# placrosse/Zaru

Measured on AMD Instinct MI355X. Metric: end-to-end faces/sec (detect+468-pt mesh), 1080p synthetic, 1/2/4/8 GPU, higher is better.
Workload: dtype f32

## Files before the change

zaru_amd/csrc/kernels/fused.hip:

```cpp
#include <algorithm>
#include <cstdio>
#include <cstdlib>

#include "../runtime/zr_kernels.h"
#include "act.h"
#include "epilogue.h"
#include "lds_dma.h"
#include "sample.h"

namespace zr {


typedef float f32x2 __attribute__((ext_vector_type(2)));
typedef float f32x4 __attribute__((ext_vector_type(4)));

constexpr int STH = 8, STW = 32;

template <int K, int S, int CO, bool PRE>
__global__ __launch_bounds__(256) void stem_kernel(const StemParams P) {
    constexpr int RIN = (STH - 1) * S + K, WIN = (STW - 1) * S + K;
    __shared__ float patch[3][RIN][WIN];
    const int tiles_x = (P.OW + STW - 1) / STW;
    const int ty0 = (blockIdx.x / tiles_x) * STH, tx0 = (blockIdx.x % tiles_x) * STW;
    const int n = blockIdx.y;
// ... 476 lines not shown
    static const bool v16 = [] {
        const char *e = std::getenv("ZARU_HIP_VALU16_VF8");
        return !e || std::strtol(e, nullptr, 10) != 0;
    }();
    const bool small = db && !((CO == 32 || (CO == 16 && v16 && p.in.W >= 96 && p.g.K >= 32)) && fit8);
    const int vf = small ? 4 : VFKC;
    const int bufsz = buf_of(vf);
    dim3 grid((ntiles + 7) / 8 * 8);
    if (db && vres) return dwpw_vres_go<K, S, CO>(p, s);
    if (db) {
        const size_t lds = 2 * sizeof(float) * (size_t)bufsz;
        if (small)
            hipLaunchKernelGGL((dwpw_valu_kernel<K, S, CO, true, 4>), grid, dim3(256), lds, s, p, tpi, ntiles, bufsz, lw);
        else
            hipLaunchKernelGGL((dwpw_valu_kernel<K, S, CO, true, VFKC>), grid, dim3(256), lds, s, p, tpi, ntiles, bufsz, lw);
    } else {
        const size_t lds = sizeof(float) * (size_t)VFKC * rmax * lw;
        hipLaunchKernelGGL((dwpw_valu_kernel<K, S, CO, false, VFKC>), grid, dim3(256), lds, s, p, tpi, ntiles, bufsz, lw);
    }
    const int vfe = db ? vf : VFKC;
    return kernel_name("dwpw_valu_kernel<%d,%d,%d,%s,%d>", K, S, CO, db ? "true" : "false", vfe);
}

template <int K, int S>
const char *dwpw_valu_co(const DwPwParams &p, hipStream_t s) {
    if (p.g.M <= 16) return dwpw_valu_go<K, S, 16>(p, s);
    if (p.g.M <= 32) return dwpw_valu_go<K, S, 32>(p, s);
    if (p.g.M <= 48) return dwpw_valu_go<K, S, 48>(p, s);
    return dwpw_valu_go<K, S, 64>(p, s);
}

}

static bool valu_form(const DwPwParams &p) {
    if (!form_on(FORM_VALU) || p.g.P < VTQ || p.in.W % 4 != 0 || p.in.W > 248 || p.g.M > 48 || p.g.K * p.g.M > 2048)
        return false;
    if (p.g.ncols % p.g.P != 0) return false;
    const int rows = (VTQ / p.OW + 2) * p.stride + p.k;
    return sizeof(float) * (size_t)VFKC * rows * (p.in.W + 8) <= 64 * 1024;
}

bool dwpw_is_vres1(const DwPwParams &p) {
    if (!valu_form(p) || p.stride != 1 || p.g.M > 32 || !form_on(FORM_VALU_DB)) return false;
    const int P = p.g.P, tpi = (P + VTQ - 1) / VTQ;
    int rmax = 0;
    for (int t = 0; t < tpi; t++) {
        const int q0 = t * VTQ, a = q0 / p.OW, b = std::min(q0 + VTQ - 1, P - 1) / p.OW;
        rmax = std::max(rmax, b - a + p.k);
    }
    const size_t buf4 = (size_t)(4 * rmax * (p.in.W + 8) + 255) / 256 * 256;
    return 2 * sizeof(float) * buf4 <= 64 * 1024 && vres_mode(p, 1, p.g.M <= 16 ? 16 : 32) == 1;
}

const char *launch_dwpw(const DwPwParams &p, hipStream_t s) {
    if (valu_form(p)) {
        if (p.k == 3) return p.stride == 1 ? dwpw_valu_co<3, 1>(p, s) : dwpw_valu_co<3, 2>(p, s);
        return p.stride == 1 ? dwpw_valu_co<5, 1>(p, s) : dwpw_valu_co<5, 2>(p, s);
    }
    return launch_dwpw_mfma(p, s);
}

const char *launch_dwpw_group(const DwPwParams *p, int n, hipStream_t s) {
    for (int i = 0; i < n; ++i)
        if (valu_form(p[i])) return nullptr;
    return launch_dwpw_mfma_group(p, n, s);
}

}
```

zaru_amd/csrc/kernels/misc.hip:

```cpp
#include <algorithm>
#include <cstdarg>
#include <cstdio>
#include <cstdlib>
#include <mutex>
#include <set>
#include <string>
#include "../runtime/zr_kernels.h"
#include "act.h"

namespace zr {

const char *kernel_name(const char *fmt, ...) {
    char buf[128];
    va_list ap;
    va_start(ap, fmt);
    vsnprintf(buf, sizeof buf, fmt, ap);
    va_end(ap);
    static std::mutex mu;
    static std::set<std::string> names;
    std::lock_guard<std::mutex> g(mu);
    return names.insert(buf).first->c_str();
}

bool form_on(Form f) {
    static const unsigned mask = [] {
        static const char *const names[FORM_COUNT] = {"dma", "v4", "valu", "valu_db", "rows", "vres", "vstore", "ws", "groups", "dwgap", "rt", "ir", "irl", "irl2", "bneck", "pin", "stemblock"};
        unsigned m = (1u << FORM_COUNT) - 1;
        const char *e = std::getenv("ZARU_HIP_FORMS");
        for (std::string s = e ? e : ""; !s.empty();) {
            const size_t comma = s.find(',');
            const std::string tok = s.substr(0, comma);
            s = comma == std::string::npos ? "" : s.substr(comma + 1);
            if (tok.size() < 2 || (tok[0] != '+' && tok[0] != '-')) continue;
            for (int i = 0; i < FORM_COUNT; i++)
                if (tok.compare(1, std::string::npos, names[i]) == 0)
                    m = tok[0] == '+' ? m | (1u << i) : m & ~(1u << i);
        }
        return m;
    }();
    return (mask >> f) & 1u;
}

__device__ __forceinline__ const float *plane_ptr(const Plane &p, int n, int c) {
    return p.p + (int64_t)n * p.sN + (int64_t)c * p.sC;
}

__global__ __launch_bounds__(256) void elt_kernel(const EltParams P) {
    const int plane = blockIdx.x;
    const int c = plane / P.N, n = plane - c * P.N;
    const int HW = P.H * P.W;
    float *dst = P.out + (int64_t)n * P.o_sN + (int64_t)c * P.o_sC;
    for (int q = blockIdx.y * blockDim.x + threadIdx.x; q < HW; q += gridDim.y * blockDim.x) {
        float v;
        if (P.op == 0) {
            v = plane_ptr(P.a, n, c)[q];
        } else if (P.op == 1) {
            v = plane_ptr(P.a, n, c)[q] + plane_ptr(P.b, n, c)[q];
        } else if (P.op == 2) {
            const int y = q / P.W, x = q - y * P.W;
            const float *s = plane_ptr(P.a, n, c) + (int64_t)(2 * y) * P.a.W + 2 * x;
            v = fmaxf(fmaxf(s[0], s[1]), fmaxf(s[P.a.W], s[P.a.W + 1]));
        } else {
            v = c < P.a.C ? plane_ptr(P.a, n, c)[q] : 0.f;
        }
        dst[q] = apply_act(P.act, v, c);
    }
}

const char *launch_elt(const EltParams &p, hipStream_t s) {
    const int HW = p.H * p.W;
    dim3 grid(p.C * p.N, std::min((HW + 255) / 256, 64));
    hipLaunchKernelGGL(elt_kernel, grid, dim3(256), 0, s, p);
    return "elt_kernel";
}

__global__ __launch_bounds__(256) void resize_kernel(const ResizeParams P) {
    const int plane = blockIdx.x;
    const int c = plane / P.N, n = plane - c * P.N;
    if (P.nact && n >= *P.nact) return;
// ... 208 lines not shown
```

zaru_amd/csrc/runtime/plan.cpp:

```cpp
#include "plan.h"

#include <algorithm>
#include <cmath>
#include <cstdlib>
#include <cstring>
#include <map>
#include <set>

namespace zr {
namespace {

struct Val {
    std::vector<int64_t> shape;
    int tensor = -1;
    int lazy = 0;
    std::string lazy_src;
    int step = -1;
    int consumers = 0;
    bool is_input = false;
    int out_idx = -1;
    int64_t out_off = 0;
    bool nhwc = false;
};

// ... 6 lines not shown
int64_t round_up(int64_t v, int64_t m) { return (v + m - 1) / m * m; }

class Compiler {
  public:
    Compiler(const OnnxModel &m, Plan &p, std::string &e) : M(m), P(p), err(e) {}

    bool run(const std::vector<uint32_t> &sel);

  private:
    const OnnxModel &M;
    Plan &P;
    std::string &err;
    std::map<std::string, Val> vals;
    std::map<std::string, int> producer;
    std::set<int> layout_nodes;
    std::vector<bool> needed;

    bool fail(const std::string &s) {
        err = s;
        return false;
    }
    const OnnxTensor *init(const std::string &n) const {
        auto it = M.inits.find(n);
        return it == M.inits.end() ? nullptr : &it->second;
    }
    Val &val(const std::string &n) { return vals[n]; }

    bool infer_shapes();
    bool trace_output(const std::string &name, int oi, int64_t off, bool nhwc);
    bool lower();
    bool lower_conv(const OnnxNode &nd);
    bool lower_gemm_node(const OnnxNode &nd);
    bool lower_act(const OnnxNode &nd);
    bool lower_add(const OnnxNode &nd);
    bool ensure_tensor(const std::string &name);
    TRef ref_of(const std::string &name);
    TRef out_ref(const std::string &name, int C, int H, int W);
    int new_storage(int64_t per_img) {
        P.storage_size.push_back(per_img);
        return (int)P.storage_size.size() - 1;
    }
    int64_t push_weights(const std::vector<float> &w) {
        int64_t off = (int64_t)P.weights.size();
        P.weights.insert(P.weights.end(), w.begin(), w.end());
        while (P.weights.size() % 4) P.weights.push_back(0.f);
        return off;
    }
    bool act_from_node(const OnnxNode &nd, int C, int Cpad, ActDesc &a);
    void finalize_outputs();
    void fuse_dw_gap();
    void group_siblings();
    void mark_inverted_residuals();
    void mark_stem_blocks();
    void allocate();
};

bool Compiler::infer_shapes() {
    for (auto &vi : M.inputs) {
        Val &v = val(vi.name);
        v.shape = vi.dims;
        if (!v.shape.empty() && v.shape[0] <= 0) v.shape[0] = 1;
        v.is_input = true;
    }
    for (auto &kv : M.inits) {
        const OnnxTensor &t = kv.second;
        if (t.dtype == 1 && (int64_t)t.f.size() != t.numel()) return fail("initializer " + kv.first + ": no f32 data");
        val(kv.first).shape = t.dims;
    }
    for (auto &vi : M.inputs)
        for (size_t i = 1; i < vi.dims.size(); i++)
            if (vi.dims[i] <= 0 || vi.dims[i] > (1 << 16)) return fail("graph input " + vi.name + ": bad dims");
    auto weight = [&](const std::string &n, size_t rank) -> const OnnxTensor * {
        const OnnxTensor *t = init(n);
        if (!t || t->dtype != 1 || t->dims.size() != rank) return nullptr;
        for (auto d : t->dims)
            if (d <= 0) return nullptr;
        return t;
    };
    for (size_t ni = 0; ni < M.nodes.size(); ni++) {
        const OnnxNode &nd = M.nodes[ni];
        const std::string &op = nd.op;
        const size_t arity = (op == "Conv" || op == "Add" || op == "PRelu" || op == "Gemm" ||
                              op == "Reshape") ? 2 : 1;
        if (nd.in.size() < arity || nd.out.empty() || nd.in[0].empty())
            return fail(op + " " + nd.name + ": missing operands");
        for (auto &i : nd.in)
            if (!i.empty() && !init(i) && (!vals.count(i) || vals[i].shape.empty()))
                return fail(op + " " + nd.name + ": operand " + i + " is not defined before use");
        for (auto &o : nd.out) producer[o] = (int)ni;
        for (auto &i : nd.in)
            if (!i.empty()) vals[i].consumers++;
        auto in = [&](int k) -> std::vector<int64_t> & { return val(nd.in[k]).shape; };
        std::vector<int64_t> s;
        if (op == "Conv") {
            auto &x = in(0);
            const OnnxTensor *w = weight(nd.in[1], 4);
            if (!w || x.size() != 4) return fail("Conv " + nd.name + ": unsupported operands");
            auto st = nd.getints("strides", {1, 1});
            auto pads = nd.getints("pads", {0, 0, 0, 0});
            const int64_t g = nd.geti("group", 1);
            if (st.size() != 2 || st[0] <= 0 || st[1] <= 0 || pads.size() != 4 ||
                *std::min_element(pads.begin(), pads.end()) < 0 || g <= 0 || x[1] != w->dims[1] * g ||
                w->dims[0] % g)
                return fail("Conv " + nd.name + ": bad strides/pads/group");
            if (nd.in.size() > 2 && !nd.in[2].empty()) {
                const OnnxTensor *b = weight(nd.in[2], 1);
// ... 707 lines not shown
    for (size_t gi = 0; gi < P.steps.size(); ++gi) {
        Step &g = P.steps[gi];
        if (g.kind != S_GAP || g.in.kind != 0 || g.in.c_off != 0) continue;
        int prod = -1, readers = 0;
        for (size_t i = 0; i < P.steps.size(); ++i) {
            const Step &s = P.steps[i];
            if (s.out.kind == 0 && s.out.id == g.in.id) prod = prod < 0 ? (int)i : -2;
            for (const TRef *r : {&s.in, &s.in2})
                if (r->kind == 0 && r->id == g.in.id) ++readers;
        }
        if (prod < 0 || readers != 1) continue;
        Step &d = P.steps[prod];
        if (d.kind != S_DW || (d.kh != 3 && d.kh != 5) || d.kh != d.kw || (int64_t)d.in.H * d.in.W > 512) continue;
        d.kind = S_DWGAP;
        d.dw_oh = d.out.H;
        d.dw_ow = d.out.W;
        d.name += "+" + g.name;
        d.out = g.out;
        d.bytes = 4.0 * ((double)d.in.C * d.in.H * d.in.W + d.in.C);
        P.steps.erase(P.steps.begin() + gi);
        --gi;
    }
}

void Compiler::mark_inverted_residuals() {
    std::vector<int> reads(P.storage_size.size(), 0);
    for (const Step &s : P.steps)
        for (const TRef *r : {&s.in, &s.in2})
            if (r->kind == 0 && r->id >= 0) reads[r->id]++;
    for (size_t i = 0; i + 1 < P.steps.size(); i++) {
        Step &e = P.steps[i];
        const Step &d = P.steps[i + 1];
        e.ir = e.kind == S_GEMM && e.group == 1 && d.group == 1 && e.KK == 1 && e.res_mode == 0 && e.out.kind == 0 &&
               e.out.c_off == 0 && e.in.kind == 0 && e.in.c_off == 0 && d.kind == S_DWPW && d.in.kind == 0 &&
               d.in.id == e.out.id && d.in.c_off == 0 && reads[e.out.id] == 1 && e.M == d.K;
    }
}

void Compiler::mark_stem_blocks() {
    std::vector<int> reads(P.storage_size.size(), 0);
    for (const Step &s : P.steps)
        for (const TRef *r : {&s.in, &s.in2})
            if (r->kind == 0 && r->id >= 0) reads[r->id]++;
    for (size_t i = 0; i + 1 < P.steps.size(); i++) {
        Step &e = P.steps[i];
        const Step &d = P.steps[i + 1];
        e.sb = e.kind == S_DIRECT && e.stem && e.M <= 32 && e.group == 1 && d.group == 1 && e.out.kind == 0 &&
               e.out.c_off == 0 && d.kind == S_DWPW && d.in.kind == 0 && d.in.id == e.out.id && d.in.c_off == 0 &&
               d.res_mode != 0 && d.in2.kind == 0 && d.in2.id == e.out.id && d.in2.c_off == 0 &&
               reads[e.out.id] == 2;
    }
}

void Compiler::group_siblings() {
    const int n = (int)P.steps.size();
    if (n < 2) return;
    auto touches = [](const TRef &r, const TRef &w) {
        return r.kind == w.kind && r.kind != 1 && r.id >= 0 && r.id == w.id;
    };
    std::vector<std::vector<char>> dep(n, std::vector<char>(n, 0));
    for (int j = 0; j < n; ++j)
        for (int i = 0; i < j; ++i) {
            const Step &a = P.steps[i], &b = P.steps[j];
            bool d = touches(b.in, a.out) || touches(b.out, a.out) || touches(b.out, a.in);
            if (b.res_mode || b.kind == S_ELT) d = d || touches(b.in2, a.out);
            if (a.res_mode || a.kind == S_ELT) d = d || touches(b.out, a.in2);
            dep[j][i] = d;
        }
    std::vector<std::vector<char>> anc = dep;
    for (int j = 0; j < n; ++j)
        for (int i = 0; i < j; ++i)
            if (anc[j][i])
                for (int k = 0; k < i; ++k) anc[j][k] |= anc[i][k];
    auto related = [&](int a, int b) { return a < b ? anc[b][a] : anc[a][b]; };
    std::vector<char> done(n, 0);
    auto ready = [&](int j) {
        if (done[j]) return false;
        for (int i = 0; i < j; ++i)
            if (dep[j][i] && !done[i]) return false;
        return true;
    };
    auto future_partner = [&](int s) {
        for (int t = 0; t < n; ++t)
            if (t != s && !done[t] && !ready(t) && !related(s, t) && groupable(P.steps[s], P.steps[t])) return true;
        return false;
    };
    std::vector<Step> out;
    out.reserve(n);
    for (int left = n; left > 0;) {
        std::vector<int> rd;
        for (int j = 0; j < n; ++j)
            if (ready(j)) rd.push_back(j);
        auto partners_of = [&](int s) {
            std::vector<int> g{s};
            for (int t : rd)
                if (t != s && (int)g.size() < ZR_GROUP_MAX && groupable(P.steps[s], P.steps[t])) g.push_back(t);
            return g;
        };
        std::vector<int> g = partners_of(rd[0]);
        if (g.size() == 1 && future_partner(rd[0]))
            for (int r : rd)
                if (r != rd[0] && !future_partner(r)) {
                    g = partners_of(r);
                    break;
                }
        for (size_t k = 0; k < g.size(); ++k) {
            Step st = P.steps[g[k]];
            st.group = k == 0 ? (int)g.size() : 0;
            out.push_back(std::move(st));
            done[g[k]] = 1;
        }
        left -= (int)g.size();
    }
    P.steps = std::move(out);
}

void Compiler::allocate() {
    const size_t ns = P.storage_size.size();
    std::vector<int> first(ns, 1 << 30), last(ns, -1);
    int time = -1;
    std::vector<int> tof(P.steps.size());
    for (size_t i = 0; i < P.steps.size(); i++) {
        const Step &s = P.steps[i];
        if (s.group != 0) ++time;
        tof[i] = time;
        for (const TRef *r : {&s.in, &s.in2, &s.out})
            if (r->kind == 0 && r->id >= 0) {
                first[r->id] = std::min(first[r->id], time);
                last[r->id] = std::max(last[r->id], time);
            }
    }
    for (size_t i = 0; i + 1 < P.steps.size(); i++) {
        if (!P.steps[i].ir && !P.steps[i].sb) continue;
        const TRef &x = P.steps[i].in, &o = P.steps[i + 1].out;
        if (x.kind == 0 && x.id >= 0) last[x.id] = std::max(last[x.id], tof[i + 1]);
        if (o.kind == 0 && o.id >= 0) first[o.id] = std::min(first[o.id], tof[i]);
    }
    std::vector<int> order(ns);
    for (size_t i = 0; i < ns; i++) order[i] = (int)i;
    std::sort(order.begin(), order.end(),
              [&](int a, int b) { return P.storage_size[a] > P.storage_size[b]; });
    P.storage_off.assign(ns, 0);
    std::vector<int> placed;
    int64_t arena = 0;
    for (int id : order) {
        if (last[id] < 0) continue;
        std::vector<std::pair<int64_t, int64_t>> busy;
        for (int o : placed)
            if (!(last[o] < first[id] || last[id] < first[o]))
                busy.push_back({P.storage_off[o], P.storage_off[o] + P.storage_size[o]});
        std::sort(busy.begin(), busy.end());
        int64_t off = 0;
        for (auto &b : busy) {
            if (off + P.storage_size[id] <= b.first) break;
            off = std::max(off, round_up(b.second, 64));
        }
        P.storage_off[id] = off;
        arena = std::max(arena, off + P.storage_size[id]);
        placed.push_back(id);
    }
    P.arena_per_image = round_up(arena, 64);
}

bool Compiler::run(const std::vector<uint32_t> &sel) {
    if (M.inputs.size() != 1) return fail("CNN plans take exactly one input");
    if (!infer_shapes()) return false;
    auto &is = val(M.inputs[0].name).shape;
    if (is.size() != 4) return fail("input must be NCHW");
    P.input_name = M.inputs[0].name;
    P.in_C = (int)is[1];
    P.in_H = (int)is[2];
    P.in_W = (int)is[3];
    std::vector<uint32_t> outs = sel;
    if (outs.empty())
        for (uint32_t i = 0; i < M.outputs.size(); i++) outs.push_back(i);
    for (size_t oi = 0; oi < outs.size(); oi++) {
        if (outs[oi] >= M.outputs.size()) return fail("output selection index out of range");
        const std::string &name = M.outputs[outs[oi]].name;
        PlanOutput po;
        po.name = name;
        po.shape = val(name).shape;
        po.per_image = per_image(po.shape);
        P.outputs.push_back(po);
    }
    for (size_t oi = 0; oi < outs.size(); oi++)
        if (!trace_output(P.outputs[oi].name, (int)oi, 0, false)) return false;
    needed.assign(M.nodes.size(), false);
    std::vector<std::string> work;
    for (auto &o : P.outputs) work.push_back(o.name);
    std::set<std::string> seen;
    while (!work.empty()) {
        std::string n = work.back();
        work.pop_back();
        if (!seen.insert(n).second) continue;
        auto it = producer.find(n);
        if (it == producer.end()) continue;
        needed[it->second] = true;
        for (auto &i : M.nodes[it->second].in)
            if (!i.empty() && !init(i)) work.push_back(i);
    }
    for (auto &kv : vals) kv.second.consumers = 0;
    for (size_t ni = 0; ni < M.nodes.size(); ni++)
        if (needed[ni])
            for (auto &i : M.nodes[ni].in)
                if (!i.empty()) vals[i].consumers++;
    if (!lower()) return false;
    for (size_t oi = 0; oi < P.outputs.size(); oi++) {
        bool written = false;
        for (auto &s : P.steps)
            if (s.out.kind == 2 && s.out.id == (int)oi) written = true;
        if (!written) return fail("output " + P.outputs[oi].name + " is never written");
    }
    for (auto &s : P.steps)
        if (s.out.kind == 2 && s.out.o_sP != 1 && s.kind != S_GEMM && s.kind != S_DWPW &&
            (int64_t)s.out.H * s.out.W > 1)
            return fail("NHWC output on a non-GEMM step (" + s.name + "): only 1x1 / dense / depthwise->1x1 "
                        "outputs can be transposed");
    for (auto &s : P.steps) {
        P.bytes_per_image += s.bytes;
        P.flops_per_image += s.flops;
    }
    P.bytes_per_image += 0;
    int readers = 0, reader = -1;
    for (size_t i = 0; i < P.steps.size(); i++)
        for (const TRef *r : {&P.steps[i].in, &P.steps[i].in2})
            if (r->kind == 1) {
                readers++;
                reader = (int)i;
            }
    P.input_fusable = readers == 1 && P.steps[reader].kind == S_DIRECT && P.steps[reader].stem;
    if (form_on(FORM_DWGAP)) fuse_dw_gap();
    if (form_on(FORM_GROUPS)) group_siblings();
    if (form_on(FORM_IR)) mark_inverted_residuals();
    if (form_on(FORM_STEMBLOCK)) mark_stem_blocks();
    allocate();
    return true;
}

}

bool compile_plan(const OnnxModel &m, const std::vector<uint32_t> &out_sel, Plan &plan,
                  std::string &err) {
    Compiler c(m, plan, err);
    return c.run(out_sel);
}

namespace {

struct Resolved {
    const float *p;
    int64_t sN, sC, sP;
};

Resolved resolve(const TRef &r, const Plan &plan, const Binding &b) {
    Resolved o{};
    const int64_t P = (int64_t)r.H * r.W;
    if (r.kind == 0) {
        o.p = b.arena + plan.storage_off[r.id] * b.Ns + (int64_t)r.c_off * P * b.Ns;
        o.sN = P;
        o.sC = P * b.Ns;
        o.sP = 1;
    } else if (r.kind == 1) {
        o.p = b.input;
        o.sN = b.in_sN;
        o.sC = b.in_sC;
        o.sP = 1;
    } else {
        o.p = b.outputs[r.id] + r.off;
        o.sN = r.o_sN;
        o.sC = r.o_sC;
        o.sP = r.o_sP;
    }
    return o;
}

Act act_of(const ActDesc &a, const float *w) {
    Act o;
    o.kind = a.kind;
    o.lo = a.lo;
    o.hi = a.hi;
    o.slope = a.slope_off >= 0 ? w + a.slope_off : nullptr;
    return o;
}

Plane plane_of(const TRef &r, const Plan &plan, const Binding &b) {
    Resolved x = resolve(r, plan, b);
    Plane p;
// ... 95 lines not shown
        StemParams sp{};
        if (pre) sp.pre = *b.pre;
        else sp.in = plane_of(s.in, plan, b);
        sp.out = const_cast<float *>(out.p);
        sp.o_sN = out.sN;
        sp.o_sC = out.sC;
        sp.IH = s.in.H;
        sp.IW = s.in.W;
        sp.OH = s.out.H;
        sp.OW = s.out.W;
        sp.N = b.N;
        sp.Cout = s.M;
        sp.k = s.kh;
        sp.stride = s.stride;
        sp.pad_t = s.pad_t;
        sp.pad_l = s.pad_l;
        sp.w = W + s.w_off;
        sp.bias = W + s.b_off;
        sp.act = act_of(s.pre, W);
        sp.nact = b.nact;
        return sp;
    };
    for (size_t si = 0; si < plan.steps.size(); ++si) {
        const Step &s = plan.steps[si];
        if (s.sb && si + 1 < plan.steps.size()) {
            const Step &s2 = plan.steps[si + 1];
            const bool pre = s.in.kind == 1 && b.pre;
            if (hook) hook->before(stream);
            const char *kname = launch_stem_dwpw(stem_of(s, pre), pre, dwpw_of(s2), stream);
            if (kname) {
                const double bytes = (pre ? s.bytes_pre : s.bytes) + s2.bytes - 8.0 * (double)s.out.C * s.out.H * s.out.W;
                if (hook) hook->after(stream, kname, bytes * b.N, (s.flops + s2.flops) * b.N);
                ++si;
                continue;
            }
            if (hook) hook->cancel();
        }
        if (s.ir && si + 1 < plan.steps.size()) {
            const Step &s2 = plan.steps[si + 1];
            const GemmParams ge = gemm_of(s);
            const DwPwParams dp = dwpw_of(s2);
            if (hook) hook->before(stream);
            const char *kname = launch_ir(ge, dp, stream);
            if (!kname) kname = launch_irl(ge, dp, stream);
            if (!kname) kname = launch_bneck(ge, dp, stream);
            if (kname) {
                const double bytes = s.bytes + s2.bytes - 8.0 * (double)s.out.C * s.out.H * s.out.W;
                if (hook) hook->after(stream, kname, bytes * b.N, (s.flops + s2.flops) * b.N);
                ++si;
                continue;
            }
            if (hook) hook->cancel();
        }
        if (s.group >= 2 && (s.kind == S_GEMM || s.kind == S_DWPW)) {
            const int ng = std::min(s.group, ZR_GROUP_MAX);
            GemmParams gp[ZR_GROUP_MAX];
            DwPwParams dp[ZR_GROUP_MAX];
            double bytes = 0, flops = 0;
            for (int k = 0; k < ng; ++k) {
                const Step &m = plan.steps[si + k];
                if (s.kind == S_GEMM) gp[k] = gemm_of(m);
                else dp[k] = dwpw_of(m);
                bytes += m.bytes * b.N;
                flops += m.flops * b.N;
            }
            if (hook) hook->before(stream);
            const char *kname = s.kind == S_GEMM ? launch_gemm_group(gp, ng, stream) : launch_dwpw_group(dp, ng, stream);
            if (kname) {
                if (hook) hook->after(stream, kname, bytes, flops);
                si += ng - 1;
                continue;
            }
            if (hook) hook->cancel();
        }
        Resolved out = resolve(s.out, plan, b);
        const char *kname = nullptr;
        if (hook) hook->before(stream);
        switch (s.kind) {
        case S_GEMM: {
            kname = launch_gemm(gemm_of(s), stream);
            break;
        }
        case S_DWPW: {
            kname = launch_dwpw(dwpw_of(s), stream);
            break;
        }
        case S_DW: {
            DwParams d{};
            d.in = plane_of(s.in, plan, b);
            d.out = const_cast<float *>(out.p);
            d.o_sN = out.sN;
            d.o_sC = out.sC;
            d.OH = s.out.H;
            d.OW = s.out.W;
            d.N = b.N;
            d.k = s.kh;
            d.stride = s.stride;
            d.pad_t = s.pad_t;
            d.pad_l = s.pad_l;
            d.w = W + s.w_off;
            d.bias = W + s.b_off;
            d.act = act_of(s.pre, W);
            kname = launch_dw(d, stream);
            break;
        }
        case S_DIRECT: {
// ... 110 lines not shown
```

zaru_amd/csrc/runtime/plan.h:

```cpp
#pragma once
#include <string>
#include <vector>

#include "onnx_model.h"
#include "zr_kernels.h"

namespace zr {

enum StepKind { S_GEMM, S_DW, S_DIRECT, S_ELT, S_RESIZE, S_GAP, S_DWPW, S_DWGAP, S_GDC };

struct TRef {
    int kind = 0;
    int id = -1;
    int C = 0, H = 1, W = 1;
    int64_t off = 0, o_sN = 0, o_sC = 0, o_sP = 1;
    int c_off = 0;
};

struct ActDesc {
    int kind = ACT_NONE;
    float lo = 0.f, hi = 0.f;
    int64_t slope_off = -1;
};

struct Step {
    StepKind kind;
    std::string name;
    TRef in, in2, out;
    int64_t w_off = -1, b_off = -1;
    ActDesc pre, post;
    int kh = 1, kw = 1, stride = 1, pad_t = 0, pad_l = 0;
    int KK = 1, M = 0, K = 0, Mpad = 0, Kpad = 0;
    int res_mode = 0, r_C = 0;
    int elt_op = 0;
    float scale_y = 1.f, scale_x = 1.f;
    int64_t dw_w_off = -1, dw_b_off = -1;
    ActDesc dw_act;
    int dw_oh = 0, dw_ow = 0;
    bool stem = false;
    double bytes = 0, flops = 0, bytes_pre = 0;
    int group = 1;
    int ir = 0;
    int sb = 0;
};

struct PlanOutput {
    std::string name;
    std::vector<int64_t> shape;
    int64_t per_image = 0;
};

struct Plan {
    std::vector<Step> steps;
    std::vector<int64_t> storage_size;
    std::vector<int64_t> storage_off;
    int64_t arena_per_image = 0;
    std::vector<float> weights;
    std::string input_name;
    int in_C = 0, in_H = 0, in_W = 0;
    std::vector<PlanOutput> outputs;
    double bytes_per_image = 0, flops_per_image = 0;
    bool input_fusable = false;
};

bool compile_plan(const OnnxModel &m, const std::vector<uint32_t> &out_sel, Plan &plan,
                  std::string &err);

struct Binding {
    int N = 0;
    int Ns = 0;
    const float *input = nullptr;
    int64_t in_sN = 0, in_sC = 0;
    float *const *outputs = nullptr;
    float *arena = nullptr;
    const float *weights = nullptr;
    const PreprocParams *pre = nullptr;
    const int *nact = nullptr;
};

struct LaunchHook {
    virtual ~LaunchHook() = default;
    virtual void before(hipStream_t s) = 0;
    virtual void after(hipStream_t s, const char *kernel, double bytes, double flops) = 0;
    virtual void cancel() {}
};

void run_plan(const Plan &plan, const Binding &b, hipStream_t stream, LaunchHook *hook = nullptr);

}
```

zaru_amd/csrc/runtime/session.cpp:

```cpp
#include <hip/hip_runtime.h>

#include <cmath>
#include <algorithm>
#include <atomic>
#include <cstdio>
#include <cstring>
#include <map>
#include <memory>
#include <mutex>
#include <string>
#include <vector>

#include "../../../include/zaru_hip.h"
#include "onnx_model.h"
#include "plan.h"
#include "zr_track.h"
#include "../kernels/procrustes_math.h"
#include "../kernels/eye_math.h"

namespace {

thread_local std::string g_err;

int set_err(int code, const std::string &msg) noexcept {
// ... 371 lines not shown
        if (!is_output) {
            if (idx != 0) return set_err(ZR_ERR_INVALID_ARGUMENT, "input index out of range");
            if (name) *name = s->plan.input_name.c_str();
            if (shape) {
                shape[0] = 1;
                shape[1] = s->plan.in_C;
                shape[2] = s->plan.in_H;
                shape[3] = s->plan.in_W;
            }
            if (rank) *rank = 4;
            return ZR_OK;
        }
        if (idx >= s->plan.outputs.size()) return set_err(ZR_ERR_INVALID_ARGUMENT, "output index out of range");
        const auto &o = s->plan.outputs[idx];
        if (name) *name = o.name.c_str();
        if (shape)
            for (size_t i = 0; i < o.shape.size() && i < 8; i++) shape[i] = i == 0 ? 1 : o.shape[i];
        if (rank) *rank = o.shape.size();
        return ZR_OK;
    });
}

int zr_plan_describe(const uint8_t *onnx, size_t len, const uint32_t *out_sel, size_t n_sel,
                     char *buf, size_t cap, size_t *needed) {
    return guarded([&]() -> int {
        if (!onnx) return set_err(ZR_ERR_INVALID_ARGUMENT, "null model");
        zr::OnnxModel m;
        std::string err;
        if (!zr::parse_onnx(onnx, len, m, err)) return set_err(ZR_ERR_MODEL, "ONNX parse error: " + err);
        zr::Plan plan;
        std::vector<uint32_t> sel(out_sel, out_sel + n_sel);
        if (!zr::compile_plan(m, sel, plan, err)) return set_err(ZR_ERR_MODEL, err);
        static const char *kinds[] = {"gemm", "dw", "direct", "elt", "resize", "gap", "dwpw", "dwgap", "gdc"};
        static const char *acts[] = {"none", "relu", "clip", "prelu", "sigmoid"};
        std::string t;
        char line[512];
        auto ref = [](const zr::TRef &r) {
            char b[96];
            snprintf(b, sizeof b, "%s%d[%dx%dx%d]", r.kind == 0 ? "t" : r.kind == 1 ? "in" : "out",
                     r.id, r.C, r.H, r.W);
            return std::string(b);
        };
        snprintf(line, sizeof line, "input %s %dx%dx%d arena_per_image=%lld weights=%zu bytes/img=%.0f flops/img=%.0f fusable=%d\n",
                 plan.input_name.c_str(), plan.in_C, plan.in_H, plan.in_W,
                 (long long)plan.arena_per_image, plan.weights.size(), plan.bytes_per_image,
                 plan.flops_per_image, plan.input_fusable ? 1 : 0);
        t += line;
        for (auto &o : plan.outputs) {
            snprintf(line, sizeof line, "output %s per_image=%lld\n", o.name.c_str(), (long long)o.per_image);
            t += line;
        }
        for (auto &st : plan.steps) {
            snprintf(line, sizeof line,
                     "%s%s in=%s out=%s k=%dx%d s=%d M=%d K=%d KK=%d pre=%s post=%s res=%d rC=%d elt=%d off=%lld oN=%lld oC=%lld oP=%lld in2=%s grp=%d ir=%d%s\n",
                     kinds[st.kind], st.stem ? " stem" : "", ref(st.in).c_str(), ref(st.out).c_str(), st.kh, st.kw, st.stride,
                     st.M, st.K, st.KK, acts[st.pre.kind], acts[st.post.kind], st.res_mode, st.r_C,
                     st.elt_op, (long long)st.out.off, (long long)st.out.o_sN, (long long)st.out.o_sC,
                     (long long)st.out.o_sP, (st.res_mode || st.kind == zr::S_ELT) ? ref(st.in2).c_str() : "-", st.group,
                     st.ir, st.sb ? " sb=1" : "");
            t += line;
        }
        if (needed) *needed = t.size() + 1;
        if (buf && cap) {
            size_t n = std::min(cap - 1, t.size());
            memcpy(buf, t.data(), n);
            buf[n] = 0;
        }
        return ZR_OK;
    });
}

int zr_profile_enable(zr_session *s, int enable) {
    return guarded([&]() -> int {
        if (int rc = check_session(s)) return rc;
        std::lock_guard<std::mutex> g(s->prof.mu);
        s->prof.on = enable != 0;
        return ZR_OK;
    });
}

int zr_profile_read(zr_session *s, char *buf, size_t cap, size_t *needed) {
    return guarded([&]() -> int {
        if (int rc = check_session(s)) return rc;
        std::lock_guard<std::mutex> g(s->prof.mu);
        struct Agg {
            size_t n = 0;
            double ms = 0, bytes = 0, flops = 0;
        };
        std::vector<std::pair<std::string, Agg>> aggs;
        for (auto &r : s->prof.recs) {
            HIP_TRY(hipEventSynchronize(r.b));
            float ms = 0.f;
            HIP_TRY(hipEventElapsedTime(&ms, r.a, r.b));
            auto it = std::find_if(aggs.begin(), aggs.end(), [&](auto &p) { return p.first == r.kernel; });
            if (it == aggs.end()) {
                aggs.push_back({r.kernel, Agg{}});
                it = aggs.end() - 1;
            }
            it->second.n++;
            it->second.ms += ms;
            it->second.bytes += r.bytes;
            it->second.flops += r.flops;
            s->prof.pool.push_back(r.a);
            s->prof.pool.push_back(r.b);
        }
        s->prof.recs.clear();
        std::string t;
        char line[256];
        for (auto &a : aggs) {
            snprintf(line, sizeof line, "%s %zu %.6f %.0f %.0f\n", a.first.c_str(), a.second.n, a.second.ms,
                     a.second.bytes, a.second.flops);
            t += line;
// ... 1239 lines not shown
```

zaru_amd/csrc/runtime/zr_kernels.h:

```cpp
#pragma once
#include <hip/hip_runtime.h>
#include <stdint.h>

namespace zr {

enum ActKind : int { ACT_NONE = 0, ACT_RELU = 1, ACT_CLIP = 2, ACT_PRELU = 3, ACT_SIGMOID = 4 };

struct Act {
    int kind = ACT_NONE;
    float lo = 0.f, hi = 0.f;
    const float *slope = nullptr;
};

struct Plane {
    const float *p;
    int64_t sN, sC;
    int C, H, W;
};

struct GemmParams {
    const float *x;
    int64_t x_sN, x_sC;
    int KK, x_sK;
    int pk, ph, x_W;
// ... 79 lines not shown
    const FrameDesc *frames;
    const ViewDesc *views;
    int nviews, OW, OH;
    int nframes;
    float lo, adjust;
    float *out;
    int64_t o_sN, o_sC;
};

struct CandParams {
    const float *logits;
    const float *boxes;
    int N, A, D, cap;
    float logit_min;
    int *count;
    float *rec;
};

struct MatchParams {
    const float *q, *g;
    int Q, G, D;
    const int32_t *valid;
    unsigned long long *keys;
    int32_t *best_idx;
    float *best_dist;
    float *dist;
};
size_t embed_match_scratch(int Q, int G);
const char *launch_embed_match(const MatchParams &p, hipStream_t s);

struct StemParams {
    Plane in;
    PreprocParams pre;
    float *out;
    int64_t o_sN, o_sC;
    int IH, IW, OH, OW, N, Cout;
    int k, stride, pad_t, pad_l;
    const float *w;
    const float *bias;
    Act act;
    const int *nact;
};

struct DwPwParams {
    GemmParams g;
    Plane in;
    int OW;
    int k, stride, pad_t, pad_l;
    const float *dw_w;
    const float *dw_b;
    Act dw_act;
};

enum Form : int { FORM_DMA, FORM_V4, FORM_VALU, FORM_VALU_DB, FORM_ROWS, FORM_VRES, FORM_VSTORE, FORM_WS, FORM_GROUPS, FORM_DWGAP, FORM_RT, FORM_IR, FORM_IRL, FORM_IRL2, FORM_BNECK, FORM_PIN, FORM_STEMBLOCK, FORM_COUNT };
bool form_on(Form f);

bool stem_supported(int cin, int k, int stride, int cout);
inline int stem_cpad(int cout) { return cout <= 32 ? 32 : 64; }
inline bool gdc_supported(int h, int w) { return h * w >= 2 && h * w <= 64; }
bool dwpw_supported(int k, int stride);

const char *kernel_name(const char *fmt, ...) __attribute__((format(printf, 1, 2)));

const char *launch_gemm(const GemmParams &p, hipStream_t s);
const char *launch_dw(const DwParams &p, hipStream_t s);
const char *launch_direct(const DirectParams &p, hipStream_t s);
const char *launch_elt(const EltParams &p, hipStream_t s);
const char *launch_resize(const ResizeParams &p, hipStream_t s);
const char *launch_gap(const GapParams &p, hipStream_t s);
const char *launch_dwgap(const DwParams &p, hipStream_t s);
const char *launch_gdc(const DwParams &p, hipStream_t s);
const char *launch_preproc(const PreprocParams &p, hipStream_t s);
const char *launch_candidates(const CandParams &p, hipStream_t s);
const char *launch_stem(const StemParams &p, bool pre, hipStream_t s);
const char *launch_dwpw(const DwPwParams &p, hipStream_t s);
const char *launch_dwpw_mfma(const DwPwParams &p, hipStream_t s);
const char *launch_dwpw_ws(const DwPwParams &p, hipStream_t s, bool launch);
constexpr int ZR_GROUP_MAX = 4;
const char *launch_gemm_group(const GemmParams *p, int n, hipStream_t s);
const char *launch_dwpw_group(const DwPwParams *p, int n, hipStream_t s);
const char *launch_dwpw_mfma_group(const DwPwParams *p, int n, hipStream_t s);
const char *launch_ir(const GemmParams &e, const DwPwParams &d, hipStream_t s);
const char *launch_irl(const GemmParams &e, const DwPwParams &d, hipStream_t s);
const char *launch_bneck(const GemmParams &e, const DwPwParams &d, hipStream_t s);

const char *launch_stem_dwpw(const StemParams &p, bool pre, const DwPwParams &d, hipStream_t s);
bool dwpw_is_vres1(const DwPwParams &p);

}
```

Baseline: 274,200.

## Fuse stride-1 and stride-2 depthwise-pointwise blocks into one downsampling kernel

Adds a kernel that runs a stride-1 3x3 depthwise+pointwise residual block and the following stride-2 3x3 depthwise+pointwise block (with max-pool residual) in a single launch. The intermediate activation stays in LDS instead of going through global memory. The planner marks eligible adjacent pairs, allocation lifetimes are extended, and execution falls back to separate launches when the shape or LDS checks fail. It trades an extra launch and the HBM round trip for heavier LDS use, lower occupancy and recomputed halo rows per tile.

```diff
diff --git a/zaru_amd/csrc/kernels/downpair.hip b/zaru_amd/csrc/kernels/downpair.hip
--- /dev/null
+++ b/zaru_amd/csrc/kernels/downpair.hip
@@ -0,0 +1,229 @@
+#include <algorithm>
+#include <cstdint>
+
+#include "../runtime/zr_kernels.h"
+#include "act.h"
+#include "lds_dma.h"
+
+namespace zr {
+
+typedef float f32x2 __attribute__((ext_vector_type(2)));
+
+template <int TH, int VF>
+struct DpGeo {
+    static constexpr int TW = 16, NO = TH * TW;
+    static constexpr int IR = 2 * TH + 1, IC = 2 * TW + 1, NI = IR * IC;
+    static constexpr int HW = TW + 1, IRS = 2 * HW, ICS = IR * IRS;
+    static constexpr int SR = IR + 2, SG = (2 * TW + 8) / 4, LW = 4 * SG;
+    static constexpr int SLOTS = VF * SR * SG, NWI = (SLOTS + 63) / 64, NM = (NWI + 3) / 4;
+    static constexpr int BUF = NWI * 256;
+    static_assert(NI <= 256 && NO <= 64 && VF % 4 == 0, "downpair tile");
+};
+
+template <int CM, int CO, int TH, int VF>
+__global__ __launch_bounds__(256) void dwpw_down_kernel(const DwPwParams A, const DwPwParams B, int tiles_x, int tpi,
+                                                        int ntiles, int ioff) {
+    static_assert(CM % 2 == 0 && CO % 8 == 0, "downpair channel groups");
+    using Geo = DpGeo<TH, VF>;
+    constexpr int DP_TH = TH, DP_TW = Geo::TW, DP_NO = Geo::NO, DP_IC = Geo::IC, DP_NI = Geo::NI, DP_HW = Geo::HW;
+    constexpr int DP_IRS = Geo::IRS, DP_ICS = Geo::ICS, DP_SR = Geo::SR, DP_SG = Geo::SG, DP_LW = Geo::LW, DP_VF = VF;
+    constexpr int DP_SLOTS = Geo::SLOTS, DP_NWI = Geo::NWI, DP_NM = Geo::NM, DP_BUF = Geo::BUF;
+    extern __shared__ __attribute__((aligned(16))) float sm[];
+    float *sI = sm + ioff;
+    const GemmParams &GA = A.g, &GB = B.g;
+    const int cpx = gridDim.x >> 3;
+    const int tile = (blockIdx.x & 7) * cpx + (blockIdx.x >> 3);
+    if (tile >= ntiles) return;
+    const int n = tile / tpi, tt = tile - n * tpi;
+    if (GA.nact && n >= *GA.nact) return;
+    const int tyt = tt / tiles_x, oy0 = tyt * DP_TH, ox0 = (tt - tyt * tiles_x) * DP_TW;
+    const int tid = threadIdx.x, lane = tid & 63, wave = __builtin_amdgcn_readfirstlane(tid >> 6);
+    const int H = A.in.H, W = A.in.W, Cin = GA.K, M1 = GA.M;
+    const int iy0 = 2 * oy0 - 1, gx0 = 2 * ox0 - 4;
+
+    int goff[DP_NM], gch[DP_NM];
+    {
+        const uint32_t nbase = (uint32_t)n * (uint32_t)A.in.sN;
+#pragma unroll
+        for (int m = 0; m < DP_NM; ++m) {
+            const int sl = (wave + 4 * m) * 64 + lane;
+            const int c = sl / (DP_SR * DP_SG), rem = sl - c * (DP_SR * DP_SG);
+            const int r = rem / DP_SG, g = rem - r * DP_SG;
+            const int iy = iy0 + r, gx = gx0 + 4 * g;
+            const bool ok = sl < DP_SLOTS && iy >= 0 && iy < H && gx >= 0 && gx < W;
+            goff[m] = ok ? (int)((uint32_t)c * (uint32_t)A.in.sC + nbase + (uint32_t)(iy * W + gx)) : -1;
+            gch[m] = c;
+        }
+    }
+    auto stage_dma = [&](int kc, float *dst) {
+        const float *base = A.in.p + (size_t)(uint32_t)kc * (uint32_t)A.in.sC;
+        const int cl = Cin - kc;
+#pragma unroll
+        for (int m = 0; m < DP_NM; ++m) {
+            const int wi = wave + 4 * m;
+            if (wi < DP_NWI) {
+                const bool ok = goff[m] >= 0 && gch[m] < cl;
+                const float *src = ok ? base + (uint32_t)goff[m] : (const float *)&zr_zero4;
+                __builtin_amdgcn_global_load_lds((const __attribute__((address_space(1))) void *)src,
+                                                 (__attribute__((address_space(3))) void *)(dst + wi * 256), 16, 0, 0);
+            }
+        }
+    };
+
+    const bool act2 = tid < DP_NI;
+    const int p = min(tid, DP_NI - 1);
+    const int ry = p / DP_IC, rx = p - ry * DP_IC;
+    const int tb = ry * DP_LW + rx + 3;
+    const int ip = ry * DP_IRS + (rx & 1) * DP_HW + (rx >> 1);
+    const int rCA = GA.r_C;
+    f32x2 acc[CM / 2];
+#pragma unroll
+    for (int i = 0; i < CM / 2; ++i) acc[i] = (f32x2)(0.f);
+    stage_dma(0, sm);
+#pragma unroll 1
+    for (int kc = 0, j = 0; kc < Cin; kc += DP_VF, ++j) {
+        const float *buf = sm + (j & 1) * DP_BUF;
+        asm volatile("s_waitcnt vmcnt(0)" ::: "memory");
+        __syncthreads();
+        if (kc + DP_VF < Cin) stage_dma(kc + DP_VF, sm + ((j + 1) & 1) * DP_BUF);
+#pragma unroll
+        for (int c = 0; c < DP_VF; ++c) {
+            const int ch = kc + c;
+            if (ch >= Cin) break;
+            const float *t0 = buf + c * (DP_SR * DP_LW) + tb;
+            float t[9], wk[10];
+#pragma unroll
+            for (int ky = 0; ky < 3; ++ky)
+#pragma unroll
+                for (int kx = 0; kx < 3; ++kx) t[ky * 3 + kx] = t0[ky * DP_LW + kx];
+#pragma unroll
+            for (int k = 0; k < 9; ++k) wk[k] = ldc(A.dw_w, ch * 9 + k);
+            wk[9] = ldc(A.dw_b, ch);
+            const __attribute__((address_space(4))) f32x2 *wp =
+                (const __attribute__((address_space(4))) f32x2 *)(GA.wt + (size_t)ch * GA.Mpad);
+            f32x2 w2[CM / 2];
+#pragma unroll
+            for (int i = 0; i < CM / 2; ++i) w2[i] = wp[i];
+            float d = wk[9];
+#pragma unroll
+            for (int k = 0; k < 9; ++k) d = __builtin_fmaf(wk[k], t[k], d);
+            if (act2 && ch < rCA) sI[ch * DP_ICS + ip] = t[4];
+#pragma unroll
+            for (int i = 0; i < CM / 2; ++i) acc[i] = __builtin_elementwise_fma(w2[i], (f32x2)(d), acc[i]);
+        }
+    }
+    {
+        float v[CM];
+#pragma unroll
+        for (int i = 0; i < CM / 2; ++i) {
+            v[2 * i] = acc[i].x + GA.bias[2 * i];
+            v[2 * i + 1] = acc[i].y + GA.bias[2 * i + 1];
+        }
+        auto chan = [](int m) { return m; };
+        apply_act_n<CM>(GA.pre, v, chan);
+#pragma unroll
+        for (int m = 0; m < CM; ++m) v[m] += act2 && m < rCA ? sI[(m < rCA ? m : 0) * DP_ICS + ip] : 0.f;
+        apply_act_n<CM>(GA.post, v, chan);
+        const bool in = 2 * oy0 + ry < H && 2 * ox0 + rx < W;
+        if (act2) {
+#pragma unroll
+            for (int m = 0; m < CM; ++m)
+                if (m < M1) sI[m * DP_ICS + ip] = in ? v[m] : 0.f;
+        }
+    }
+    __syncthreads();
+
+    const int ty = lane / DP_TW, tx = lane - ty * DP_TW;
+    const bool act3 = lane < DP_NO;
+    const int o = min(lane, DP_NO - 1);
+    const int pb = 2 * min(ty, DP_TH - 1) * DP_IRS + tx;
+    float *sD = sm;
+#pragma unroll 1
+    for (int ch = wave; ch < M1; ch += 4) {
+        const float *t0 = sI + ch * DP_ICS + pb;
+        float t[9], wk[10];
+#pragma unroll
+        for (int ky = 0; ky < 3; ++ky)
+#pragma unroll
+            for (int kx = 0; kx < 3; ++kx) t[ky * 3 + kx] = t0[ky * DP_IRS + (kx & 1) * DP_HW + (kx >> 1)];
+#pragma unroll
+        for (int k = 0; k < 9; ++k) wk[k] = ldc(B.dw_w, ch * 9 + k);
+        wk[9] = ldc(B.dw_b, ch);
+        float d = wk[9];
+#pragma unroll
+        for (int k = 0; k < 9; ++k) d = __builtin_fmaf(wk[k], t[k], d);
+        if (act3) sD[ch * DP_NO + o] = d;
+    }
+    __syncthreads();
+    constexpr int CQ = CO / 4;
+    const int m0 = wave * CQ;
+    f32x2 a2[CQ / 2];
+#pragma unroll
+    for (int i = 0; i < CQ / 2; ++i) a2[i] = (f32x2)(0.f);
+#pragma unroll 2
+    for (int ch = 0; ch < M1; ++ch) {
+        const float d = sD[ch * DP_NO + o];
+        const __attribute__((address_space(4))) f32x2 *wp =
+            (const __attribute__((address_space(4))) f32x2 *)(GB.wt + (size_t)ch * GB.Mpad + m0);
+#pragma unroll
+        for (int i = 0; i < CQ / 2; ++i) a2[i] = __builtin_elementwise_fma(wp[i], (f32x2)(d), a2[i]);
+    }
+    float v[CQ];
+#pragma unroll
+    for (int i = 0; i < CQ / 2; ++i) {
+        v[2 * i] = a2[i].x + ldc(GB.bias, m0 + 2 * i);
+        v[2 * i + 1] = a2[i].y + ldc(GB.bias, m0 + 2 * i + 1);
+    }
+    auto chan = [m0](int r) { return m0 + r; };
+    apply_act_n<CQ>(GB.pre, v, chan);
+    const int rCB = GB.r_C;
+#pragma unroll
+    for (int r = 0; r < CQ; ++r) {
+        const bool has = m0 + r < rCB;
+        const float *t0 = sI + (has ? m0 + r : 0) * DP_ICS + pb;
+        const float pm = fmaxf(fmaxf(t0[0], t0[DP_HW]), fmaxf(t0[DP_IRS], t0[DP_IRS + DP_HW]));
+        v[r] += has ? pm : 0.f;
+    }
+    apply_act_n<CQ>(GB.post, v, chan);
+    const int OW = B.OW, OH = GB.P / OW, oy = oy0 + ty, ox = ox0 + tx;
+    if (!act3 || oy >= OH || ox >= OW) return;
+    const uint32_t ob = (uint32_t)n * (uint32_t)GB.o_sN + (uint32_t)(oy * OW + ox) * (uint32_t)GB.o_sP;
+#pragma unroll
+    for (int r = 0; r < CQ; ++r)
+        if (m0 + r < GB.M) GB.out[ob + (uint32_t)(m0 + r) * (uint32_t)GB.o_sC] = v[r];
+}
+
+namespace {
+
+template <int CM, int CO, int TH, int VF>
+const char *down_go(const DwPwParams &a, const DwPwParams &b, hipStream_t s) {
+    using Geo = DpGeo<TH, VF>;
+    if (a.g.Mpad < CM || b.g.Mpad < CO) return nullptr;
+    const int OW = b.OW, OH = b.g.P / OW, N = b.g.ncols / b.g.P;
+    const int tiles_x = (OW + Geo::TW - 1) / Geo::TW, tpi = tiles_x * ((OH + TH - 1) / TH);
+    const int ntiles = tpi * N;
+    dim3 grid((ntiles + 7) / 8 * 8);
+    const int ioff = std::max((a.g.K > VF ? 2 : 1) * Geo::BUF, (a.g.M * Geo::NO + 3) / 4 * 4);
+    const size_t lds = sizeof(float) * ((size_t)ioff + ((size_t)a.g.M * Geo::ICS + 3) / 4 * 4);
+    if (lds > 64 * 1024) return nullptr;
+    hipLaunchKernelGGL((dwpw_down_kernel<CM, CO, TH, VF>), grid, dim3(256), lds, s, a, b, tiles_x, tpi, ntiles, ioff);
+    return kernel_name("dwpw_down_kernel<%d,%d,%d,%d>", CM, CO, TH, VF);
+}
+
+}
+
+const char *launch_down_pair(const DwPwParams &a, const DwPwParams &b, hipStream_t s) {
+    const GemmParams &ga = a.g, &gb = b.g;
+    if (!form_on(FORM_DOWN) || a.k != 3 || b.k != 3 || dwpw_vres_case(a) != 1 || dwpw_vres_case(b) != 2) return nullptr;
+    if (b.in.p != ga.out || b.in.sN != ga.o_sN || b.in.sC != ga.o_sC || ga.o_sP != 1 || b.in.H != a.in.H ||
+        b.in.W != a.in.W || gb.K != ga.M || ga.K > ga.M || ga.r_C > ga.K || ga.nact != gb.nact || ga.ncols / ga.P != gb.ncols / gb.P ||
+        ga.Mpad % 2 != 0 || gb.Mpad % 2 != 0 || ((uintptr_t)ga.wt | (uintptr_t)gb.wt) % 8 != 0)
+        return nullptr;
+    const int cm = std::max(ga.K, ga.M);
+    if (cm <= 16 && gb.M <= 32) return down_go<16, 32, 3, 4>(a, b, s);
+    if (cm <= 32 && gb.M <= 32) return down_go<32, 32, 3, 4>(a, b, s);
+    if (cm <= 48 && gb.M <= 48) return down_go<48, 48, 3, 4>(a, b, s);
+    return nullptr;
+}
+
+}
diff --git a/zaru_amd/csrc/kernels/fused.hip b/zaru_amd/csrc/kernels/fused.hip
--- a/zaru_amd/csrc/kernels/fused.hip
+++ b/zaru_amd/csrc/kernels/fused.hip
@@ -552,6 +552,19 @@
     return 2 * sizeof(float) * buf4 <= 64 * 1024 && vres_mode(p, 1, p.g.M <= 16 ? 16 : 32) == 1;
 }
 
+int dwpw_vres_case(const DwPwParams &p) {
+    if (!valu_form(p) || !form_on(FORM_VALU_DB) || (p.k != 3 && p.k != 5) || (p.stride != 1 && p.stride != 2)) return 0;
+    const int P = p.g.P, tpi = (P + VTQ - 1) / VTQ;
+    int rmax = 0;
+    for (int t = 0; t < tpi; t++) {
+        const int q0 = t * VTQ, a = q0 / p.OW, b = std::min(q0 + VTQ - 1, P - 1) / p.OW;
+        rmax = std::max(rmax, (b - a) * p.stride + p.k);
+    }
+    const size_t buf4 = (size_t)(4 * rmax * (p.in.W + 8) + 255) / 256 * 256;
+    if (2 * sizeof(float) * buf4 > 64 * 1024) return 0;
+    return vres_mode(p, p.stride, p.g.M <= 16 ? 16 : p.g.M <= 32 ? 32 : 48);
+}
+
 const char *launch_dwpw(const DwPwParams &p, hipStream_t s) {
     if (valu_form(p)) {
         if (p.k == 3) return p.stride == 1 ? dwpw_valu_co<3, 1>(p, s) : dwpw_valu_co<3, 2>(p, s);
diff --git a/zaru_amd/csrc/kernels/misc.hip b/zaru_amd/csrc/kernels/misc.hip
--- a/zaru_amd/csrc/kernels/misc.hip
+++ b/zaru_amd/csrc/kernels/misc.hip
@@ -24,7 +24,7 @@
 
 bool form_on(Form f) {
     static const unsigned mask = [] {
-        static const char *const names[FORM_COUNT] = {"dma", "v4", "valu", "valu_db", "rows", "vres", "vstore", "ws", "groups", "dwgap", "rt", "ir", "irl", "irl2", "bneck", "pin", "stemblock"};
+        static const char *const names[FORM_COUNT] = {"dma", "v4", "valu", "valu_db", "rows", "vres", "vstore", "ws", "groups", "dwgap", "rt", "ir", "irl", "irl2", "bneck", "pin", "stemblock", "down"};
         unsigned m = (1u << FORM_COUNT) - 1;
         const char *e = std::getenv("ZARU_HIP_FORMS");
         for (std::string s = e ? e : ""; !s.empty();) {
diff --git a/zaru_amd/csrc/runtime/plan.cpp b/zaru_amd/csrc/runtime/plan.cpp
--- a/zaru_amd/csrc/runtime/plan.cpp
+++ b/zaru_amd/csrc/runtime/plan.cpp
@@ -82,6 +82,7 @@
     void group_siblings();
     void mark_inverted_residuals();
     void mark_stem_blocks();
+    void mark_down_pairs();
     void allocate();
 };
 
@@ -895,6 +896,25 @@
     }
 }
 
+void Compiler::mark_down_pairs() {
+    std::vector<int> reads(P.storage_size.size(), 0);
+    for (const Step &s : P.steps)
+        for (const TRef *r : {&s.in, &s.in2})
+            if (r->kind == 0 && r->id >= 0) reads[r->id]++;
+    auto dw3 = [](const Step &s, int stride) {
+        return s.kind == S_DWPW && s.group == 1 && s.kh == 3 && s.kw == 3 && s.stride == stride &&
+               s.dw_act.kind == ACT_NONE;
+    };
+    for (size_t i = 0; i + 1 < P.steps.size(); i++) {
+        Step &a = P.steps[i];
+        const Step &b = P.steps[i + 1];
+        a.dp = dw3(a, 1) && dw3(b, 2) && a.res_mode == 1 && a.in.kind == 0 && a.in2.kind == 0 && a.in2.id == a.in.id &&
+               a.in2.c_off == a.in.c_off && a.out.kind == 0 && a.out.c_off == 0 &&
+               b.in.kind == 0 && b.in.id == a.out.id && b.in.c_off == 0 && b.res_mode == 2 && b.in2.kind == 0 &&
+               b.in2.id == a.out.id && b.in2.c_off == 0 && b.pad_t == 0 && b.pad_l == 0 && reads[a.out.id] == 2;
+    }
+}
+
 void Compiler::group_siblings() {
     const int n = (int)P.steps.size();
     if (n < 2) return;
@@ -974,7 +994,7 @@
             }
     }
     for (size_t i = 0; i + 1 < P.steps.size(); i++) {
-        if (!P.steps[i].ir && !P.steps[i].sb) continue;
+        if (!P.steps[i].ir && !P.steps[i].sb && !P.steps[i].dp) continue;
         const TRef &x = P.steps[i].in, &o = P.steps[i + 1].out;
         if (x.kind == 0 && x.id >= 0) last[x.id] = std::max(last[x.id], tof[i + 1]);
         if (o.kind == 0 && o.id >= 0) first[o.id] = std::min(first[o.id], tof[i]);
@@ -1076,6 +1096,7 @@
     if (form_on(FORM_GROUPS)) group_siblings();
     if (form_on(FORM_IR)) mark_inverted_residuals();
     if (form_on(FORM_STEMBLOCK)) mark_stem_blocks();
+    if (form_on(FORM_DOWN)) mark_down_pairs();
     allocate();
     return true;
 }
@@ -1277,6 +1298,19 @@
             }
             if (hook) hook->cancel();
         }
+        if (s.dp && si + 1 < plan.steps.size()) {
+            const Step &s2 = plan.steps[si + 1];
+            const DwPwParams da = dwpw_of(s), db = dwpw_of(s2);
+            if (hook) hook->before(stream);
+            const char *kname = launch_down_pair(da, db, stream);
+            if (kname) {
+                const double bytes = s.bytes + s2.bytes - 8.0 * (double)s.out.C * s.out.H * s.out.W;
+                if (hook) hook->after(stream, kname, bytes * b.N, (s.flops + s2.flops) * b.N);
+                ++si;
+                continue;
+            }
+            if (hook) hook->cancel();
+        }
         if (s.group >= 2 && (s.kind == S_GEMM || s.kind == S_DWPW)) {
             const int ng = std::min(s.group, ZR_GROUP_MAX);
             GemmParams gp[ZR_GROUP_MAX];
diff --git a/zaru_amd/csrc/runtime/plan.h b/zaru_amd/csrc/runtime/plan.h
--- a/zaru_amd/csrc/runtime/plan.h
+++ b/zaru_amd/csrc/runtime/plan.h
@@ -42,6 +42,7 @@
     int group = 1;
     int ir = 0;
     int sb = 0;
+    int dp = 0;
 };
 
 struct PlanOutput {
diff --git a/zaru_amd/csrc/runtime/session.cpp b/zaru_amd/csrc/runtime/session.cpp
--- a/zaru_amd/csrc/runtime/session.cpp
+++ b/zaru_amd/csrc/runtime/session.cpp
@@ -447,12 +447,12 @@
         }
         for (auto &st : plan.steps) {
             snprintf(line, sizeof line,
-                     "%s%s in=%s out=%s k=%dx%d s=%d M=%d K=%d KK=%d pre=%s post=%s res=%d rC=%d elt=%d off=%lld oN=%lld oC=%lld oP=%lld in2=%s grp=%d ir=%d%s\n",
+                     "%s%s in=%s out=%s k=%dx%d s=%d M=%d K=%d KK=%d pre=%s post=%s res=%d rC=%d elt=%d off=%lld oN=%lld oC=%lld oP=%lld in2=%s grp=%d ir=%d%s%s\n",
                      kinds[st.kind], st.stem ? " stem" : "", ref(st.in).c_str(), ref(st.out).c_str(), st.kh, st.kw, st.stride,
                      st.M, st.K, st.KK, acts[st.pre.kind], acts[st.post.kind], st.res_mode, st.r_C,
                      st.elt_op, (long long)st.out.off, (long long)st.out.o_sN, (long long)st.out.o_sC,
                      (long long)st.out.o_sP, (st.res_mode || st.kind == zr::S_ELT) ? ref(st.in2).c_str() : "-", st.group,
-                     st.ir, st.sb ? " sb=1" : "");
+                     st.ir, st.sb ? " sb=1" : "", st.dp ? " dp=1" : "");
             t += line;
         }
         if (needed) *needed = t.size() + 1;
diff --git a/zaru_amd/csrc/runtime/zr_kernels.h b/zaru_amd/csrc/runtime/zr_kernels.h
--- a/zaru_amd/csrc/runtime/zr_kernels.h
+++ b/zaru_amd/csrc/runtime/zr_kernels.h
@@ -155,7 +155,7 @@
     Act dw_act;
 };
 
-enum Form : int { FORM_DMA, FORM_V4, FORM_VALU, FORM_VALU_DB, FORM_ROWS, FORM_VRES, FORM_VSTORE, FORM_WS, FORM_GROUPS, FORM_DWGAP, FORM_RT, FORM_IR, FORM_IRL, FORM_IRL2, FORM_BNECK, FORM_PIN, FORM_STEMBLOCK, FORM_COUNT };
+enum Form : int { FORM_DMA, FORM_V4, FORM_VALU, FORM_VALU_DB, FORM_ROWS, FORM_VRES, FORM_VSTORE, FORM_WS, FORM_GROUPS, FORM_DWGAP, FORM_RT, FORM_IR, FORM_IRL, FORM_IRL2, FORM_BNECK, FORM_PIN, FORM_STEMBLOCK, FORM_DOWN, FORM_COUNT };
 bool form_on(Form f);
 
 bool stem_supported(int cin, int k, int stride, int cout);
@@ -189,5 +189,7 @@
 
 const char *launch_stem_dwpw(const StemParams &p, bool pre, const DwPwParams &d, hipStream_t s);
 bool dwpw_is_vres1(const DwPwParams &p);
+int dwpw_vres_case(const DwPwParams &p);
+const char *launch_down_pair(const DwPwParams &a, const DwPwParams &b, hipStream_t s);
 
 }
```

New measurement: 274,500 (median of 3 runs). No clear change (+0.1%).
